# TheShadow29/vognet-pytorch

Hardware: AMD Instinct MI355X
Metric: queries/sec (VOGNet forward, gt5 spat, bs=4) (higher is better)
Workload: dtype bf16; 1 GPU; VOGNet spat gt5 (obj_tx+mul_tx, use_rel) bs=4; global_batch=4, batch_per_gpu=4, sentence_len=12, batches_in_flight=4, lang_cobatch=1, lstm=persistent layer kernel (1 launch per layer), submission=hipGraph on 4 HIP streams, weights=seeded default-init-like, vocab 5000, launches_per_forward=see kernels_usec (--full): steps joined by '+' share one launch (csrc/pair.hip)

## Files before the change

### include/vog_hip.h

```cpp
#ifndef VOG_HIP_H
#define VOG_HIP_H

#include <stddef.h>
#include <stdint.h>

#ifdef __cplusplus
extern "C" {
#endif

#define VOG_ABI_VERSION 1

typedef enum { VOG_BF16 = 0, VOG_F16 = 1 } vog_dtype;
typedef enum { VOG_MDL_IGRND = 0, VOG_MDL_VGRND = 1, VOG_MDL_VOG = 2 } vog_mdl_kind;
typedef enum { VOG_CONC_SEP = 0, VOG_CONC_TEMP = 1, VOG_CONC_SPAT = 2 } vog_conc_type;

int vog_version(void);
const char* vog_last_error(void);


struct vog_vislang_args;
typedef struct vog_gemm_args {
  const void* a; int a_is_f32; int64_t lda; const int32_t* a_rows;
  const void* w; int64_t ldw;
  const float* bias;
// ... 131 lines not shown
int vog_lang_prep(void* zero, int64_t zero_bytes, int64_t ones_bytes, const int64_t* words_ind, const int64_t* word_mask,
                  const int64_t* lens, int32_t* tok, int32_t* rows, int Bn, int T, int nsrl,
                  int seq_len, int vocab_size,
                  const void* emb16, void* a0_frag, int emb_dim, void* stream);

typedef struct vog_visprep_args {
  const float* src0; void* dst0; int64_t n0; const float* src1; void* dst1; int64_t n1; vog_dtype dtype;
  const float* props; int n_rows; float vid_w, vid_h;
  const float* w_pe0; float* u0; int H0; float nfrm_div0;
  const float* w_pe1; float* u1; int H1; float nfrm_div1;
} vog_visprep_args;
int vog_vis_prep(const vog_visprep_args* a, void* stream);
int vog_prep_fused(void* zero, int64_t zero_bytes, int64_t ones_bytes, const int64_t* words_ind, const int64_t* word_mask,
                   const int64_t* lens, int32_t* tok, int32_t* rows, int Bn, int T, int nsrl,
                   int seq_len, int vocab_size, const void* emb16, void* a0_frag, int emb_dim,
                   const vog_visprep_args* vis, void* stream);

typedef struct vog_lstm_step_args {
  const float* gx; const void* whh; const void* h_in; void* h_out; float* c;
  void* out16; const int64_t* lens; int Bn, T, R, step; vog_dtype dtype;
  int out_frag; int final_row0;
} vog_lstm_step_args;
int vog_bilstm_step(const vog_lstm_step_args* a, void* stream);
typedef struct vog_lstm_layer_args {
  const float* gxs; const void* whh; void* hx; uint32_t* sync; void* out16;
  const int64_t* lens; int Bn, T, R; vog_dtype dtype;
  int out_frag;
  const void* wih; const void* xa; const float* bias; int K;
  uint32_t* fault; int inject_stall;
  const float* gx_table; const int32_t* tok;
} vog_lstm_layer_args;
int vog_bilstm_layer_supported(int Bn, int R);
int vog_bilstm_fused_cols(void);
int64_t vog_bilstm_hx_bytes(int Bn, int T, int R);
int vog_bilstm_layer(const vog_lstm_layer_args* a, void* stream);

int vog_lstm_pack_whh(const float* whh_fwd, const float* whh_bwd, void* dst_host, int R, vog_dtype dtype);
int vog_lstm_pack_w(const float* w_fwd, const float* w_bwd, void* dst_host, int R, int K, vog_dtype dtype);

int vog_srl_argvec(const float* full, const int64_t* capture, const int64_t* inds_msk,
                   const float* w, const float* bias, float* lang,
                   int Bn, int T, int nsrl, int L, void* stream);

typedef struct vog_vislang_args {
  const float* vis; const float* lang; float* x32; void* x16;
  int n_vid, nfrm, nppf, nsrl, dv, dl; int lang_per_vid;
  int nc_v; vog_dtype dtype;
} vog_vislang_args;
int vog_vislang_layout(const vog_vislang_args* a, void* stream);

typedef struct vog_score_args {
  const float* h1; const float* w2; const float* b2;
  const int64_t* arg_msk; const int64_t* cmp_msk;
  float* outs; float* outs_eval;
  int n_vid, nfrm, nppf, nsrl, dh; int conc_type; int ncmp, nc_v, nvl, nfrm0, nppf0;
} vog_score_args;
int vog_score_head(const vog_score_args* a, void* stream);

typedef struct vog_predcmp_args {
  const float* final_hidden;
  const float* prop_seg;
  const float* w0; const float* b0; const float* w2; const float* b2;
  const float* outs;
  const int64_t* arg_msk; const int64_t* cmp_msk; const int64_t* verb_ind;
  float* vidf_outs; float* fin_scores_loss; float* fin_scores;
  int B, ncmp, nvl, nsrl, NP, nfrm0, nppf0, L, dp0, dps;
// ... 402 lines not shown
```

### vognet-pytorch_amd/csrc/lstm.hip

```cpp
#include <stdlib.h>
#include "lstm_dev.h"
#include "wpack_dev.h"
#include "pair_ids.h"

namespace vog {

__global__ void lstm_schedule_kernel(const int64_t* __restrict__ lens, int32_t* __restrict__ rows,
                                     int Bn, int T) {
  const int i = blockIdx.x * blockDim.x + threadIdx.x;
  if (i >= Bn * T) return;
  const int b = i / T, t = i % T;
  const int len = (int)lens[b];
  rows[i] = t < len ? t * Bn + b : -1;
  rows[Bn * T + i] = t < len ? T * Bn - 1 + (len - 1 - t) * Bn + b : -1;
}

const void* kid_lstm_layer_f16() { return reinterpret_cast<const void*>(lstm_layer_kernel<F16, 32>); }

int lstm_step_run(const vog_lstm_step_args* a, hipStream_t st) {
  VOG_CHECK_ARG(a && a->gx && a->whh && a->h_in && a->h_out && a->c && a->out16 && a->lens);
  VOG_CHECK_ARG(a->Bn > 0 && a->T > 0 && a->R > 0 && (a->R % 32) == 0 && a->step >= 0 && a->step < a->T);
  VOG_CHECK_ARG(a->h_in != a->h_out);
  LstmParams p{a->gx, (const unsigned short*)a->whh, (const unsigned short*)a->h_in,
               (unsigned short*)a->h_out, a->c, (unsigned short*)a->out16, a->lens,
               a->Bn, a->T, a->R, a->step, a->out_frag, a->final_row0, 0};
  static const int dbg = perf_env("VOG_LSTM_DEBUG") ? atoi(perf_env("VOG_LSTM_DEBUG")) : 0;
  p.debug = dbg;
  dim3 grid(ceil_div(a->R, 4), 2);
  VOG_DISPATCH_DTYPE(a->dtype, ::vog::launch((lstm_step_kernel<T16>), grid, dim3(256), 0, st, p));
  VOG_LAUNCH_CHECK();
  return 0;
}

}

extern "C" int vog_bilstm_step(const vog_lstm_step_args* a, void* stream) {
  return vog::lstm_step_run(a, (hipStream_t)stream);
}

extern "C" int vog_bilstm_layer_supported(int Bn, int R) {
  const int ks = R / 32;
  return Bn >= 1 && Bn <= 16 && R % 32 == 0 && R / 32 <= 64 && (ks == 1 || ks == 2 || ks == 4 || ks == 32);
}

extern "C" int vog_bilstm_fused_cols(void) { return 16 * vog::LstmLayerBody<vog::F16, 32>::NCT_MAX; }

extern "C" int64_t vog_bilstm_hx_bytes(int Bn, int T, int R) {
  if (Bn <= 0 || T <= 0 || R <= 0) return -1;
  return (int64_t)T * 2 * Bn * R * 2;
}

extern "C" int vog_bilstm_layer(const vog_lstm_layer_args* a, void* stream) {
  VOG_CHECK_ARG(a && (a->gxs || a->wih || a->gx_table) && a->whh && a->hx && a->sync && a->out16 && a->lens && a->T > 0);
  VOG_CHECK_ARG(!a->gx_table || (a->tok && a->Bn * a->T <= vog::LstmLayerBody<vog::F16, 32>::TOK_MAX));
  if (!vog_bilstm_layer_supported(a->Bn, a->R))
    VOG_FAIL(-1, "persistent BiLSTM layer: unsupported Bn=%d R=%d (use vog_bilstm_step)", a->Bn, a->R);
  vog::LstmLayerParams p{a->gxs, (const unsigned short*)a->whh, (unsigned short*)a->hx, a->sync,
                         (unsigned short*)a->out16, a->lens, a->Bn, a->T, a->R, a->out_frag,
                         (const unsigned short*)a->wih, (const unsigned short*)a->xa, a->bias, a->K,
                         a->fault, a->inject_stall, 0, a->gx_table, a->tok};
  if (const char* e = vog::perf_env("VOG_LSTM_HALF_PROJ")) p.half_proj = atoi(e);
  const bool fused = a->wih != nullptr && !a->gx_table;
  if (a->gx_table) p.wih = nullptr;
  if (fused) VOG_CHECK_ARG(a->xa && a->bias && a->K > 0 && (a->K % 256) == 0 && a->Bn * a->T <= vog_bilstm_fused_cols());
  dim3 grid(a->R / 32, 2);
  hipStream_t st = (hipStream_t)stream;
  size_t lds_extra = 0;
  if (const char* e = vog::perf_env("VOG_LSTM_LDS_EXTRA")) lds_extra = (size_t)atoi(e);
#define VOG_LAUNCH_LAYER(KS)                                                                          \
  VOG_DISPATCH_DTYPE(a->dtype, {                                                                      \
    auto kern = vog::lstm_layer_kernel<T16, KS>;                                                      \
    using Body = vog::LstmLayerBody<T16, KS>;                                                         \
    static bool attr_set = false;                                                                     \
    if (!attr_set) {                                                                                  \
      VOG_HIP(hipFuncSetAttribute(reinterpret_cast<const void*>(kern),                                \
                                  hipFuncAttributeMaxDynamicSharedMemorySize, 156 * 1024));          \
      attr_set = true;                                                                                \
    }                                                                                                 \
    ::vog::launch(kern, grid, dim3(512),                                                              \
                  (fused ? Body::lds_fused(a->Bn, a->Bn * a->T) : Body::lds_plain(a->Bn)) + lds_extra, st, p); \
  })
  switch (a->R / 32) {
    case 1: VOG_LAUNCH_LAYER(1); break;
    case 2: VOG_LAUNCH_LAYER(2); break;
    case 4: VOG_LAUNCH_LAYER(4); break;
    default: VOG_LAUNCH_LAYER(32); break;
  }
#undef VOG_LAUNCH_LAYER
  VOG_LAUNCH_CHECK();
  return 0;
}

extern "C" int vog_lstm_schedule(const int64_t* lens, int32_t* rows, int Bn, int T, void* stream) {
  VOG_CHECK_ARG(lens && rows && Bn > 0 && T > 0);
  ::vog::launch(vog::lstm_schedule_kernel, dim3(vog::ceil_div(Bn * T, 128)), dim3(128), 0,
                     (hipStream_t)stream, lens, rows, Bn, T);
  VOG_LAUNCH_CHECK();
  return 0;
}

extern "C" int vog_lstm_pack_whh(const float* whh_fwd, const float* whh_bwd, void* dst_host, int R,
                                 vog_dtype dtype) {
  return vog_lstm_pack_w(whh_fwd, whh_bwd, dst_host, R, R, dtype);
}

extern "C" int vog_lstm_pack_w(const float* whh_fwd, const float* whh_bwd, void* dst_host, int R, int K,
                               vog_dtype dtype) {
  VOG_CHECK_ARG(whh_fwd && whh_bwd && dst_host && R > 0 && (R % 4) == 0 && K > 0 && (K % 32) == 0);
  unsigned short* dst = (unsigned short*)dst_host;
  for (int64_t g = 0; g < (int64_t)8 * R * K / 8; ++g) {
    int n, k;
    vog::wpack_lstm_src(g, R, K, &n, &k);
    const float* src = (n < 4 * R ? whh_fwd : whh_bwd) + (int64_t)(n % (4 * R)) * K + k;
    unsigned short* d = dst + g * 8;
    for (int j = 0; j < 8; ++j) {
      if (dtype == VOG_BF16) {
        unsigned int u; memcpy(&u, &src[j], 4);
        u += 0x7fffu + ((u >> 16) & 1u);
        d[j] = (unsigned short)(u >> 16);
      } else {
        _Float16 h = (_Float16)src[j];
// ... 7 lines not shown
```

### vognet-pytorch_amd/csrc/lstm_dev.h

```cpp
#pragma once
#include "common.h"

namespace vog {

struct LstmParams {
  const float* gxs; const unsigned short* whh; const unsigned short* h_in; unsigned short* h_out;
  float* c; unsigned short* out16; const int64_t* lens;
  int Bn, T, R, step; int out_frag, final_row0; int debug;
};

__device__ __forceinline__ float sigm(float x) { return 1.0f / (1.0f + __expf(-x)); }
__device__ __forceinline__ float sigm_fast(float x) { return __builtin_amdgcn_rcpf(1.0f + __expf(-x)); }
__device__ __forceinline__ float tanh_fast(float x) {
  const float a = fabsf(x);
  const float e = __expf(-2.0f * a);
  const float t = (1.0f - e) * __builtin_amdgcn_rcpf(1.0f + e);
  return x < 0.f ? -t : t;
}
__device__ __forceinline__ float tanh_(float x) {
  const float a = fabsf(x);
  const float e = __expf(-2.0f * a);
  const float t = (1.0f - e) / (1.0f + e);
  return x < 0.f ? -t : t;
}
// ... 90 lines not shown
    VOG_TS(2);
  }
}

struct LstmLayerParams {
  const float* gxs; const unsigned short* whh; unsigned short* hx; unsigned int* sync;
  unsigned short* out16; const int64_t* lens; int Bn, T, R; int out_frag;
  const unsigned short* wih; const unsigned short* xa; const float* bias; int K;
  unsigned int* fault; int inject_stall;
  int half_proj;
  const float* gxtab; const int32_t* tok;
};

#define VOG_RLX_AGENT __ATOMIC_RELAXED, __HIP_MEMORY_SCOPE_AGENT
#define VOG_RLX_WG __ATOMIC_RELAXED, __HIP_MEMORY_SCOPE_WORKGROUP


__device__ __forceinline__ u32x4 load16_l2(const void* base, unsigned byte_off, unsigned bytes) {
  const __amdgpu_buffer_rsrc_t r = __builtin_amdgcn_make_buffer_rsrc(const_cast<void*>(base), 0, (int)bytes, 0x00020000);
  return __builtin_amdgcn_raw_buffer_load_b128(r, (int)byte_off, 0, 16 );
}
__device__ __forceinline__ bool has_unwritten(u32x4 v) {
  unsigned m = 0;
#pragma unroll
  for (int i = 0; i < 4; ++i) { const unsigned y = ~v[i]; m |= (y - 0x00010001u) & v[i] & 0x80008000u; }
  return m != 0;
}
__device__ __forceinline__ unsigned xcc_id() {
  unsigned x;
  asm volatile("s_getreg_b32 %0, hwreg(HW_REG_XCC_ID)" : "=s"(x));
  return x & 15u;
}

template <typename T16, int KSTEPS>
struct LstmLayerBody {
  using Params = LstmLayerParams;
  static constexpr int THREADS = 512;
  static constexpr int RW = KSTEPS * 32, HS_LD = RW + 32;
  static constexpr int GX_PITCH = 20;
  static constexpr int NCT_MAX = 5;
  static constexpr size_t gx_bytes(int ncols) { return (size_t)8 * ((ncols + 15) / 16 * 16) * GX_PITCH * 4; }
  static constexpr size_t GX_BYTES = gx_bytes(16 * NCT_MAX);
  static constexpr size_t hs_bytes(int Bn) { return ((size_t)2 * Bn * HS_LD * 2 + 15) / 16 * 16; }
  static constexpr size_t xbuf_bytes(int ncols) { return (size_t)2 * ((ncols + 15) / 16) * 8 * 1024; }
  static constexpr int TOK_MAX = 16 * 24;
  static constexpr size_t TAIL = 16 + 16 * 32 * 2 + TOK_MAX * 4;
  static constexpr size_t lds_plain(int Bn) { return hs_bytes(Bn) + TAIL; }
  static constexpr size_t lds_fused(int Bn, int ncols) {
    return gx_bytes(ncols) + (hs_bytes(Bn) > xbuf_bytes(ncols) ? hs_bytes(Bn) : xbuf_bytes(ncols)) + TAIL;
  }
  static constexpr size_t LDS_MAX = GX_BYTES + ((size_t)2 * 16 * HS_LD * 2 > (size_t)2 * NCT_MAX * 8 * 1024 ? (size_t)2 * 16 * HS_LD * 2 : (size_t)2 * NCT_MAX * 8 * 1024) + TAIL;

  static __device__ __forceinline__ void run(const LstmLayerParams& p, const BlockCtx& cx, unsigned char* smem) {
    const int tid = threadIdx.x, lane = tid & 63;
    const int wid = __builtin_amdgcn_readfirstlane(tid >> 6);
    const int dir = cx.by;
    const int R = p.R;
    const int tile0 = cx.bx * 8 + wid;
    const int b = lane & 15, ul = lane >> 4, kg = (lane >> 4) * 8;
    const bool valid_b = b < p.Bn;
    const int len = valid_b ? (int)p.lens[b] : 0;
    const bool fused = p.wih != nullptr;
    const int ncols = p.Bn * p.T;
    const int gx_cols = (ncols + 15) / 16 * 16;
    unsigned char* uni = smem + (fused ? gx_bytes(ncols) : 0);
    unsigned short* hs = reinterpret_cast<unsigned short*>(uni);
    const size_t uni_bytes = fused ? (hs_bytes(p.Bn) > xbuf_bytes(ncols) ? hs_bytes(p.Bn) : xbuf_bytes(ncols)) : hs_bytes(p.Bn);
    unsigned int* flags = reinterpret_cast<unsigned int*>(uni + uni_bytes);
    unsigned short* pub = reinterpret_cast<unsigned short*>(uni + uni_bytes + 16);
    int* tokl = reinterpret_cast<int*>(uni + uni_bytes + 16 + 16 * 32 * 2);
    const bool tab = p.gxtab != nullptr;
    const int unit0 = tile0 * 4 + ul;
    auto load_tab = [&](int s2, float (&g)[4], const int* tk) __attribute__((always_inline)) {
      int row = 0;
      const bool on = valid_b && s2 < len && s2 < p.T;
      if (on) row = tk[b * p.T + (dir == 0 ? s2 : len - 1 - s2)];
      const float4 v = *reinterpret_cast<const float4*>(p.gxtab + (((int64_t)row * 2 + dir) * R + unit0) * 4);
      g[0] = v.x; g[1] = v.y; g[2] = v.z; g[3] = v.w;
    };
    float gtA[4] = {0.f, 0.f, 0.f, 0.f}, gtB[4] = {0.f, 0.f, 0.f, 0.f}, gtC[4] = {0.f, 0.f, 0.f, 0.f};
    if (tab) {
      load_tab(0, gtA, p.tok);
      load_tab(1, gtB, p.tok);
      load_tab(2, gtC, p.tok);
      for (int i = tid; i < p.Bn * p.T; i += THREADS) tokl[i] = p.tok[i];
    }

    if (tid == 0) {
      flags[0] = 0;
      __hip_atomic_fetch_add(p.sync + 16 + dir * 16 + xcc_id(), 1u, VOG_RLX_AGENT);
    }

    float c = 0.f, h_own = 0.f;
    VOG_TSL(p.T, 0);
    float* gxl = reinterpret_cast<float*>(smem) + (size_t)wid * gx_cols * GX_PITCH;
    if (fused) {
      unsigned char* xch = uni;
      const int nct = (ncols + 15) >> 4;
      const int ksteps = p.K >> 5;
      const int nchunk = (p.half_proj && p.K >= 2048) ? (ksteps >> 4) : (ksteps >> 3);
      f32x4 ga[NCT_MAX];
#pragma unroll
      for (int ct = 0; ct < NCT_MAX; ++ct) ga[ct] = f32x4{0.f, 0.f, 0.f, 0.f};
      const u16x8* wsrc = reinterpret_cast<const u16x8*>(p.wih) + (((int64_t)dir * (R / 4) + tile0) * ksteps) * 64 + lane;
      const uint4* xsrc = reinterpret_cast<const uint4*>(p.xa);
      unsigned char* xbuf[2] = {xch, xch + nct * 8 * 1024};
      auto load_w = [&](u16x8 (&wq)[8], int c) {
#pragma unroll
        for (int ks = 0; ks < 8; ++ks) wq[ks] = wsrc[(c * 8 + ks) * 64];
      };
      auto dma_x = [&](int c) {
#pragma unroll
        for (int j = 0; j < NCT_MAX; ++j) {
          const int piece = j * 8 + wid;
          const int ct = piece >> 3, r = ((piece & 7) << 6) + lane;
          __builtin_amdgcn_global_load_lds(
              (const __attribute__((address_space(1))) void*)(xsrc + ((int64_t)(ct < nct ? ct : 0) * ksteps + c * 8) * 64 + r),
              (__attribute__((address_space(3))) void*)(xbuf[c & 1] + (ct < nct ? piece : (piece & 7)) * 1024), 16, 0, 0);
        }
      };
      auto mfmas = [&](const u16x8 (&wq)[8], int c) {
        const unsigned char* xb = xbuf[c & 1];
#pragma unroll
        for (int ct = 0; ct < NCT_MAX; ++ct)
          if (ct < nct) {
#pragma unroll
            for (int ks = 0; ks < 8; ++ks) {
              const u16x8 xf = *reinterpret_cast<const u16x8*>(xb + ((ct * 8 + ks) * 64 + lane) * 16);
              ga[ct] = mfma16<T16>(wq[ks], xf, ga[ct]);
            }
          }
      };
      u16x8 w0[8], w1[8];
      dma_x(0); load_w(w0, 0);
      if (nchunk > 1) { dma_x(1); load_w(w1, 1); }
      for (int c = 0; c < nchunk; c += 2) {
        if (c + 1 < nchunk) asm volatile("s_waitcnt vmcnt(%0)" ::"n"(NCT_MAX + 8) : "memory");
        else asm volatile("s_waitcnt vmcnt(0)" ::: "memory");
        __syncthreads();
        mfmas(w0, c);
        __syncthreads();
        if (c + 2 < nchunk) { dma_x(c + 2); load_w(w0, c + 2); }
        if (c + 1 < nchunk) {
          if (c + 2 < nchunk) asm volatile("s_waitcnt vmcnt(%0)" ::"n"(NCT_MAX + 8) : "memory");
          else asm volatile("s_waitcnt vmcnt(0)" ::: "memory");
          __syncthreads();
          mfmas(w1, c + 1);
          __syncthreads();
          if (c + 3 < nchunk) { dma_x(c + 3); load_w(w1, c + 3); }
        }
      }
      float bs[4];
#pragma unroll
      for (int r = 0; r < 4; ++r) bs[r] = p.bias[(int64_t)dir * 4 * R + (int64_t)r * R + tile0 * 4 + ul];
#pragma unroll
      for (int ct = 0; ct < NCT_MAX; ++ct)
        if (ct < nct)
          *reinterpret_cast<float4*>(gxl + (ct * 16 + b) * GX_PITCH + ul * 4) =
              make_float4(ga[ct][0] + bs[0], ga[ct][1] + bs[1], ga[ct][2] + bs[2], ga[ct][3] + bs[3]);
    }
    VOG_TSL(p.T, 1);
    u16x8 wf[KSTEPS];
#pragma unroll
    for (int ks = 0; ks < KSTEPS; ++ks)
      wf[ks] = *reinterpret_cast<const u16x8*>(
          p.whh + ((((int64_t)dir * (R / 4) + tile0) * KSTEPS + ks) * 64 + lane) * 8);
    bool dead = false;
    if (tid == 0) {
      unsigned spins = 0, nz = 0;
      for (;;) {
        unsigned sum = 0;
        nz = 0;
#pragma unroll
        for (int x = 0; x < 16; ++x) {
          const unsigned v = __hip_atomic_load(p.sync + 16 + dir * 16 + x, VOG_RLX_AGENT);
          sum += v;
          nz += v != 0 ? 1u : 0u;
        }
        if (sum >= cx.gx) break;
        __builtin_amdgcn_s_sleep(2);
        if (++spins > (1u << 20) || __hip_atomic_load(p.sync + 2, VOG_RLX_AGENT) != 0) {
          __hip_atomic_store(p.sync + 2, 1u, VOG_RLX_AGENT);
          flags[0] = 1;
          nz = 2;
          break;
        }
      }
      flags[1] = nz == 1 ? 1u : 0u;
    }
    __syncthreads();
    const bool same_xcd = flags[1] != 0;
    dead = flags[0] != 0 || p.inject_stall == 1 || (p.inject_stall == 2 && dir == 1);

    const unsigned hx_bytes = (unsigned)((size_t)p.T * 2 * p.Bn * R * 2);
    const int cps = RW / 8;
    const int nchunks = p.Bn * cps;
    const int hs_buf = p.Bn * HS_LD;

    for (int s = 0; s < p.T; ++s) {
      VOG_TSL(s, 0);
      float gin[4] = {0.f, 0.f, 0.f, 0.f};
      if (tab) {
#pragma unroll
        for (int r = 0; r < 4; ++r) { gin[r] = gtA[r]; gtA[r] = gtB[r]; gtB[r] = gtC[r]; }
        if (s == 0) load_tab(3, gtC, tokl);
      } else
      if (fused) {
        if (valid_b && s < len) {
          const int pos_in = dir == 0 ? s : len - 1 - s;
          const float4 g4 = *reinterpret_cast<const float4*>(gxl + (b * p.T + pos_in) * GX_PITCH + ul * 4);
          gin[0] = g4.x; gin[1] = g4.y; gin[2] = g4.z; gin[3] = g4.w;
        }
      } else {
#pragma unroll
        for (int r = 0; r < 4; ++r)
          gin[r] = valid_b ? p.gxs[(((int64_t)dir * p.T + s) * p.Bn + b) * 4 * R + (int64_t)r * R + tile0 * 4 + ul] : 0.f;
      }
      f32x4 acc0 = f32x4{0.f, 0.f, 0.f, 0.f}, acc1 = f32x4{0.f, 0.f, 0.f, 0.f};
      if (s > 0) {
        unsigned short* hsb = hs + (s & 1) * hs_buf;
        const unsigned slot_off = (unsigned)(((size_t)(s - 1) * 2 + dir) * p.Bn * R * 2);
        constexpr int MAXR = 4;
#ifndef VOG_LSTM_INFL
#define VOG_LSTM_INFL 4
#endif
        constexpr int INFL = VOG_LSTM_INFL;
        u32x4 vq[INFL];
        const int sb0 = tid / cps, j0 = tid - sb0 * cps;
        const unsigned off0 = slot_off + (unsigned)(sb0 * R + j0 * 8) * 2;
        const unsigned off_step = (unsigned)((THREADS / cps) * R) * 2;
        const int lds0 = sb0 * HS_LD + j0 * 8, lds_step = (THREADS / cps) * HS_LD;
        static_assert(THREADS % (RW / 8) == 0 || (RW / 8) % THREADS == 0, "hand-off fetch: chunk stride");
#pragma unroll
        for (int r0 = 0; r0 < MAXR; r0 += INFL) {
#pragma unroll
        for (int q = 0; q < INFL; ++q)
          if (tid + (r0 + q) * THREADS < nchunks) vq[q] = load16_l2(p.hx, off0 + (r0 + q) * off_step, hx_bytes);
#pragma unroll
        for (int q = 0; q < INFL; ++q) {
          const int r = r0 + q;
// ... 85 lines not shown
        } else {
          if (valid_b) pub[b * 32 + wid * 4 + ul] = x0;
          __syncthreads();
          if (tid < p.Bn * 4) {
            const int sb = tid >> 2, q = tid & 3;
            const u32x4 v = *reinterpret_cast<const u32x4*>(pub + sb * 32 + q * 8);
            u32x4* dst = reinterpret_cast<u32x4*>(slot + (size_t)sb * R + cx.bx * 32 + q * 8);
            asm volatile("global_store_dwordx4 %0, %1, off sc1" :: "v"(dst), "v"(v) : "memory");
          }
        }
      }
      VOG_TSL(s, 4);
    }
    if (dead && p.fault && tid == 0 &&
        __hip_atomic_exchange(p.sync + 3, 1u, __ATOMIC_RELAXED, __HIP_MEMORY_SCOPE_AGENT) == 0u)
      __hip_atomic_fetch_add(p.fault, 1u, __ATOMIC_RELAXED, __HIP_MEMORY_SCOPE_SYSTEM);
    if (valid_b) {
      const int unit = tile0 * 4 + ul;
      const unsigned short v = dead ? (unsigned short)0x7fff : to16<T16>(h_own);
      if (p.out_frag) p.out16[frag_a(p.Bn * p.T + b, dir * R + unit, 2 * R)] = v;
      else p.out16[((int64_t)p.Bn * p.T + b) * 2 * R + (int64_t)dir * R + unit] = v;
      if (dead)
        for (int t = 0; t < p.T; ++t) {
          if (p.out_frag) p.out16[frag_a(b * p.T + t, dir * R + unit, 2 * R)] = (unsigned short)0x7fff;
          else p.out16[((int64_t)b * p.T + t) * 2 * R + (int64_t)dir * R + unit] = (unsigned short)0x7fff;
        }
    }
  }
};

#ifndef VOG_LSTM_KATTR
#define VOG_LSTM_KATTR
#endif
template <typename T16, int KSTEPS>
__global__ __launch_bounds__(512) VOG_LSTM_KATTR void lstm_layer_kernel(LstmLayerParams p) {
  extern __shared__ __attribute__((aligned(16))) unsigned char lstm_smem[];
  LstmLayerBody<T16, KSTEPS>::run(p, BlockCtx{blockIdx.x, blockIdx.y, gridDim.x, gridDim.y}, lstm_smem);
}

}
```

### vognet-pytorch_amd/csrc/pair.hip

```cpp
#include <functional>
#include <map>
#include <mutex>
#include <utility>
#include "gemm_dev.h"
#include "lstm_dev.h"
#include "txtail_dev.h"
#include "visenc_dev.h"
#include "qkvrb_dev.h"
#include <tuple>
#include "pair_ids.h"

#ifndef VOG_VS_PAIR_DEPTH
#define VOG_VS_PAIR_DEPTH 2
#endif

namespace vog {

thread_local std::vector<LaunchRecord>* g_pair_capture = nullptr;

template <typename A, typename B>
__global__ __launch_bounds__((A::THREADS > B::THREADS ? A::THREADS : B::THREADS))
void pair_kernel(typename A::Params a, typename B::Params b, unsigned nA, unsigned gax, unsigned gay,
                 unsigned gbx, unsigned gby, unsigned delay_b) {
  extern __shared__ __attribute__((aligned(1024))) unsigned char pair_smem[];
// ... 17 lines not shown
      ra.arg_bytes != sizeof(typename A::Params) || rb.arg_bytes != sizeof(typename B::Params))
    VOG_FAIL(-1, "pair launch: recorded launches do not match the registered bodies");
  typename A::Params pa; typename B::Params pb;
  memcpy(&pa, ra.args, sizeof(pa));
  memcpy(&pb, rb.args, sizeof(pb));
  const unsigned nA = ra.grid[0] * ra.grid[1], nB = rb.grid[0] * rb.grid[1];
  const size_t lds = ra.dyn_lds > rb.dyn_lds ? ra.dyn_lds : rb.dyn_lds;
  if (lds > 156 * 1024) VOG_FAIL(-1, "pair launch: %zu bytes of LDS", lds);
  auto kern = pair_kernel<A, B>;
  static bool attr_set = false;
  if (!attr_set) {
    VOG_HIP(hipFuncSetAttribute(reinterpret_cast<const void*>(kern), hipFuncAttributeMaxDynamicSharedMemorySize,
                                156 * 1024));
    attr_set = true;
  }
  static const unsigned delay_b = perf_env("VOG_PAIR_DELAY") ? (unsigned)atoi(perf_env("VOG_PAIR_DELAY")) : 0u;
  ::vog::launch(kern, dim3(nA + nB), dim3(MAXT), lds, st, pa, pb, nA, ra.grid[0], ra.grid[1], rb.grid[0], rb.grid[1], delay_b);
  VOG_LAUNCH_CHECK();
  return 0;
}

using SkinnyIh = GemmSkinnyBody<F16, false, 4, 1, 4>;
using SkinnyRow = GemmSkinnyRowBody<F16, 8>;
template <typename B>
static int launch_pair_outproj(const LaunchRecord& ra, const LaunchRecord& rb, hipStream_t st) {
  GemmParams pa;
  if (ra.arg_bytes == sizeof(pa)) {
    memcpy(&pa, ra.args, sizeof(pa));
    if (SkinnyRow::fits(pa, ra.grid[1])) return launch_pair<SkinnyRow, B>(ra, rb, st);
  }
  return launch_pair<SkinnyIh, B>(ra, rb, st);
}

static constexpr int kPairDeclined = 1;
static std::map<std::pair<const void*, const void*>, PairFn>& registry() {
  static std::map<std::pair<const void*, const void*>, PairFn> r;
  static std::once_flag once;
  std::call_once(once, [] {
    using Lstm = LstmLayerBody<F16, 32>;
    r[{kid_lstm_layer_f16(), kid_vis_enc_f16()}] = &launch_pair<Lstm, VisEncBody<F16>>;
    r[{kid_lstm_layer_f16(), kid_vis_enc_stream_f16()}] = &launch_pair<Lstm, VisEncStreamBody<F16, VOG_VS_PAIR_DEPTH>>;
    r[{kid_lstm_layer_f16(), kid_gemm_pipe_qkv(VOG_BF16)}] = &launch_pair<Lstm, GemmPipeBody<BF16, 64, 64, 2, EPI_QKV>>;
    r[{kid_lstm_layer_f16(), kid_gemm_pipe_qkv(VOG_F16)}] = &launch_pair<Lstm, GemmPipeBody<F16, 64, 64, 2, EPI_QKV>>;
    r[{kid_lstm_layer_f16(), kid_tx_tail_512(VOG_BF16)}] = &launch_pair<Lstm, TxTailBody<BF16, F16, 2, false, 0>>;
    r[{kid_lstm_layer_f16(), kid_tx_tail_512(VOG_F16)}] = &launch_pair<Lstm, TxTailBody<F16, F16, 2, false, 0>>;
    r[{kid_lstm_layer_f16(), kid_vis_enc_stream_split_f16()}] = &launch_pair<Lstm, VisEncStreamBody<F16, VOG_VS_DEPTH, true>>;
    r[{kid_lstm_layer_f16(), kid_tx_tail_split_512_f16()}] = &launch_pair<Lstm, TxTailBody<F16, F16, 2, false, 0, 1, true>>;
    r[{kid_gemm_skinny_f16(), kid_gemm_pipe_qkv_split_f16()}] = &launch_pair_outproj<GemmPipeBody<F16, 64, 64, 2, EPI_QKV, true>>;
    r[{kid_gemm_skinny_f16(), kid_gemm_pipe_qkv(VOG_BF16)}] = &launch_pair_outproj<GemmPipeBody<BF16, 64, 64, 2, EPI_QKV>>;
    r[{kid_gemm_skinny_f16(), kid_gemm_pipe_qkv(VOG_F16)}] = &launch_pair_outproj<GemmPipeBody<F16, 64, 64, 2, EPI_QKV>>;
    r[{kid_gemm_pipe_plain3_f16(), kid_gemm_pipe_qkv(VOG_BF16)}] = &launch_pair<GemmPipeBody<F16, 64, 64, 3, EPI_PLAIN>, GemmPipeBody<BF16, 64, 64, 2, EPI_QKV>>;
    r[{kid_gemm_pipe_plain3_f16(), kid_gemm_pipe_qkv(VOG_F16)}] = &launch_pair<GemmPipeBody<F16, 64, 64, 3, EPI_PLAIN>, GemmPipeBody<F16, 64, 64, 2, EPI_QKV>>;
  });
  return r;
}

int pair_launch(const std::function<int(hipStream_t)>& fa, const std::function<int(hipStream_t)>& fb,
                hipStream_t st, bool* fused) {
  if (fused) *fused = false;
  std::vector<LaunchRecord> recs;
  if (g_pair_capture) { VOG_TRY(fa(st)); return fb(st); }
  g_pair_capture = &recs;
  int rc = fa(st);
  const size_t na = recs.size();
  if (rc == 0) rc = fb(st);
  g_pair_capture = nullptr;
  if (rc != 0) return rc;
  if (na == 1 && recs.size() == 2) {
    auto it = registry().find({recs[0].host_fn, recs[1].host_fn});
    if (it != registry().end()) {
      const int prc = it->second(recs[0], recs[1], st);
      if (prc != kPairDeclined) {
        if (fused) *fused = prc == 0;
        return prc;
      }
    }
  }
  VOG_TRY(fa(st));
  return fb(st);
}
// ... 3 lines not shown
```

### vognet-pytorch_amd/csrc/pair_ids.h

```cpp
#pragma once
namespace vog {
const void* kid_gemm_skinny_f16();
const void* kid_gemm_skinny_wide_f16();
const void* kid_gemm_skinny_f32a_short(int dtype);
const void* kid_gemm_pipe_qkv(int dtype);
const void* kid_gemm_pipe_plain3_f16();
const void* kid_lstm_layer_f16();
const void* kid_tx_tail_512(int dtype);
const void* kid_vis_enc_f16();
const void* kid_vis_enc_stream_f16();
const void* kid_gemm_pipe_qkv_split_f16();
const void* kid_tx_tail_split_512_f16();
const void* kid_vis_enc_stream_split_f16();
}
```

### vognet-pytorch_amd/lib.py

```python
from __future__ import annotations

import ctypes as C
import os
from typing import Optional

_HERE = os.path.dirname(os.path.abspath(__file__))
LIB_PATH = os.environ.get("VOG_HIP_LIB") or os.path.join(_HERE, "csrc", "libvog_hip.so")

VOG_BF16, VOG_F16 = 0, 1
MDL_KIND = {"igrnd": 0, "vgrnd": 1, "vog": 2}
CONC_TYPE = {"sep": 0, "svsq": 0, "temp": 1, "spat": 2}
DTYPE = {"bf16": VOG_BF16, "f16": VOG_F16, "fp16": VOG_F16}

c_i32, c_i64, c_f32, c_vp = C.c_int, C.c_int64, C.c_float, C.c_void_p


class VogError(RuntimeError):
    pass


class GemmArgs(C.Structure):
    _fields_ = [("a", c_vp), ("a_is_f32", c_i32), ("lda", c_i64), ("a_rows", c_vp),
                ("w", c_vp), ("ldw", c_i64), ("bias", c_vp), ("residual", c_vp), ("ldr", c_i64),
                ("c32", c_vp), ("c16", c_vp), ("ldc", c_i64), ("ldc16", c_i64),
# ... 324 lines not shown

AVG_EMA, AVG_SWA = 1, 2


class OptAvgTensor(C.Structure):
    _fields_ = [("avg", c_vp), ("p", c_vp), ("n", c_i64)]


class OptAvgState(C.Structure):
    _fields_ = [("n_averaged", c_i32), ("updated", c_i32), ("w", c_f32), ("reserved", c_i32)]


class OptAvgArgs(C.Structure):
    _fields_ = [("tensors", C.POINTER(OptAvgTensor)), ("n_tensors", c_i32), ("mode", c_i32), ("decay", C.c_double),
                ("warmup", c_i32), ("start", c_i32), ("every", c_i32), ("opt_state", c_vp), ("step", c_i32), ("state", c_vp)]


class Batch(C.Structure):
    _fields_ = [("B", c_i32), ("ncmp", c_i32), ("T", c_i32),
                ("srl_arg_words_ind", c_vp), ("srl_arg_word_mask", c_vp),
                ("srl_arg_word_mask_len", c_vp), ("srl_arg_words_capture", c_vp),
                ("srl_arg_inds_msk", c_vp), ("num_cmp_msk", c_vp), ("verb_ind_in_srl", c_vp),
                ("pad_region_feature", c_vp), ("seg_feature_for_frms", c_vp), ("pad_proposals", c_vp),
                ("mdl_outs", c_vp), ("mdl_outs_eval", c_vp), ("vidf_outs", c_vp),
                ("fin_scores_loss", c_vp), ("fin_scores", c_vp), ("pred_rec", c_vp),
                ("shared_lang", c_vp), ("shared_final_hidden", c_vp), ("fault", c_vp), ("obj_out", c_vp), ("stats", c_vp),
                ("enc_prop", c_vp), ("enc_seg", c_vp)]


SYMBOLS = {
    "vog_version": (c_i32, []),
    "vog_ctx_split_supported": (c_i32, [c_vp, c_i32]),
    "vog_bilstm_fused_cols": (c_i32, []),
    "vog_last_error": (C.c_char_p, []),
    "vog_gemm_bias_act": (c_i32, [C.POINTER(GemmArgs), c_vp]),
    "vog_pack_w_frag": (c_i32, [c_vp, c_i64, c_i32, c_i32, c_vp, c_i32]),
    "vog_pack_w_frag32": (c_i32, [c_vp, c_i64, c_i32, c_i32, c_vp, c_i32]),
    "vog_tx_tail_supported": (c_i32, [c_i32, c_i32, c_i32]),
    "vog_tx_tail_scratch_bytes": (c_i64, [c_i32, c_i32]),
    "vog_tx_tail_fwd": (c_i32, [C.POINTER(TxTailArgs), c_vp]),
    "vog_encoder_layer_fwd": (c_i32, [C.POINTER(EncoderLayerArgs), c_vp]),
    "vog_vis_encode_supported": (c_i32, [c_i32, c_i32, c_i32, c_i32]),
    "vog_vis_encode": (c_i32, [C.POINTER(VisencArgs), c_vp]),
    "vog_seg_replicate": (c_i32, [C.POINTER(VisencArgs), c_vp]),
    "vog_vis_concat": (c_i32, [C.POINTER(VisconcatArgs), c_vp]),
    "vog_obj_restore": (c_i32, [C.POINTER(ObjrestoreArgs), c_vp]),
    "vog_loss_scratch_bytes": (c_i64, [C.POINTER(LossArgs)]),
    "vog_loss_fwd": (c_i32, [C.POINTER(LossArgs), c_vp]),
    "vog_loss_bwd": (c_i32, [C.POINTER(LossArgs), c_vp, c_vp, c_vp]),
    "vog_assemble_batch": (c_i32, [C.POINTER(AssembleArgs), c_vp]),
    "vog_assemble_from_bank": (c_i32, [C.POINTER(BankAssembleArgs), c_vp]),
    "vog_splitk_finish": (c_i32, [C.POINTER(SplitkProb), C.POINTER(SplitkProb), c_vp]),
    "vog_qkv_proj": (c_i32, [C.POINTER(QkvArgs), c_vp]),
    "vog_qkv_rowblock_supported": (c_i32, [c_i32, c_i32]),
    "vog_qkv_combine": (c_i32, [C.POINTER(QkvCombArgs), c_vp]),
    "vog_rel_attention_fwd": (c_i32, [C.POINTER(AttnArgs), c_vp]),
    "vog_rel_attention_struct_fwd": (c_i32, [C.POINTER(AttnStructArgs), c_vp]),
    "vog_residual_layernorm": (c_i32, [c_vp, c_vp, c_vp, c_vp, c_vp, c_i32, c_i32, c_i32, c_vp]),
    "vog_cast_f32_to_t16": (c_i32, [c_vp, c_vp, c_i64, c_vp, c_vp, c_i64, c_i32, c_vp]),
    "vog_box_u": (c_i32, [c_vp, c_vp, c_vp, c_i32, c_i32, c_f32, c_f32, c_f32, c_vp]),
    "vog_srl_gather": (c_i32, [c_vp, c_vp, c_vp, c_i32, c_i32, c_i32, c_i32, c_i32, c_vp]),
    "vog_bilstm_layer_supported": (c_i32, [c_i32, c_i32]),
    "vog_mul_tail_bwd_scratch_bytes": (c_i64, [c_i32, c_i32, c_i32, c_i32]),
    "vog_mul_tail_bwd": (c_i32, [C.POINTER(TailBwdArgs), c_vp]),
    "vog_attn_f32_scratch_bytes": (c_i64, [c_i32, c_i32, c_i32, c_i32]),
    "vog_attn_f32": (c_i32, [C.POINTER(AttnF32Args), c_vp]),
# ... 131 lines not shown
```

Baseline: 65630 queries/s.

## Specialize fused BiLSTM projection on column-tile count and stage x through registers

Makes the number of projection column tiles a template parameter of the persistent BiLSTM layer kernel, with one instantiation per tile count, so the register accumulators and MFMA loops are sized exactly and runtime guards disappear. The input-projection x operand is now loaded into registers and written to LDS instead of using global_load_lds DMA with explicit vmcnt waits. The K loop is restructured to drop one barrier per chunk and adds sched_barrier hints plus optional nontemporal weight loads. The pairing registry is extended to cover every instantiation. This costs more compiled kernel variants, and register staging of x raises register pressure.

```diff
diff --git a/include/vog_hip.h b/include/vog_hip.h
--- a/include/vog_hip.h
+++ b/include/vog_hip.h
@@ -187,6 +187,7 @@
 } vog_lstm_layer_args;
 int vog_bilstm_layer_supported(int Bn, int R);
 int vog_bilstm_fused_cols(void);
+int vog_bilstm_fused_tiles(int cols);
 int64_t vog_bilstm_hx_bytes(int Bn, int T, int R);
 int vog_bilstm_layer(const vog_lstm_layer_args* a, void* stream);
 
diff --git a/vognet-pytorch_amd/csrc/lstm.hip b/vognet-pytorch_amd/csrc/lstm.hip
--- a/vognet-pytorch_amd/csrc/lstm.hip
+++ b/vognet-pytorch_amd/csrc/lstm.hip
@@ -15,7 +15,22 @@
   rows[Bn * T + i] = t < len ? T * Bn - 1 + (len - 1 - t) * Bn + b : -1;
 }
 
-const void* kid_lstm_layer_f16() { return reinterpret_cast<const void*>(lstm_layer_kernel<F16, 32>); }
+int lstm_layer_nct(int cols) {
+  constexpr int NCT_MAX = LstmLayerBody<F16, 32>::NCT_MAX;
+  return cols >= 1 && cols <= 16 * NCT_MAX ? (cols + 15) / 16 : 0;
+}
+
+const void* kid_lstm_layer_f16(int nct) {
+  switch (nct) {
+    case 0: return reinterpret_cast<const void*>(lstm_layer_kernel<F16, 32, 0>);
+    case 1: return reinterpret_cast<const void*>(lstm_layer_kernel<F16, 32, 1>);
+    case 2: return reinterpret_cast<const void*>(lstm_layer_kernel<F16, 32, 2>);
+    case 3: return reinterpret_cast<const void*>(lstm_layer_kernel<F16, 32, 3>);
+    case 4: return reinterpret_cast<const void*>(lstm_layer_kernel<F16, 32, 4>);
+    case 5: return reinterpret_cast<const void*>(lstm_layer_kernel<F16, 32, 5>);
+    default: return nullptr;
+  }
+}
 
 int lstm_step_run(const vog_lstm_step_args* a, hipStream_t st) {
   VOG_CHECK_ARG(a && a->gx && a->whh && a->h_in && a->h_out && a->c && a->out16 && a->lens);
@@ -45,6 +60,11 @@
 
 extern "C" int vog_bilstm_fused_cols(void) { return 16 * vog::LstmLayerBody<vog::F16, 32>::NCT_MAX; }
 
+extern "C" int vog_bilstm_fused_tiles(int cols) {
+  const int nct = vog::lstm_layer_nct(cols);
+  return nct > 0 ? nct : -1;
+}
+
 extern "C" int64_t vog_bilstm_hx_bytes(int Bn, int T, int R) {
   if (Bn <= 0 || T <= 0 || R <= 0) return -1;
   return (int64_t)T * 2 * Bn * R * 2;
@@ -63,14 +83,16 @@
   const bool fused = a->wih != nullptr && !a->gx_table;
   if (a->gx_table) p.wih = nullptr;
   if (fused) VOG_CHECK_ARG(a->xa && a->bias && a->K > 0 && (a->K % 256) == 0 && a->Bn * a->T <= vog_bilstm_fused_cols());
+  const int nct = fused ? vog::lstm_layer_nct(a->Bn * a->T) : 0;
+  if (fused && nct == 0) VOG_FAIL(-1, "persistent BiLSTM layer: no fused instantiation for %d columns", a->Bn * a->T);
   dim3 grid(a->R / 32, 2);
   hipStream_t st = (hipStream_t)stream;
   size_t lds_extra = 0;
   if (const char* e = vog::perf_env("VOG_LSTM_LDS_EXTRA")) lds_extra = (size_t)atoi(e);
-#define VOG_LAUNCH_LAYER(KS)                                                                          \
+#define VOG_LAUNCH_LAYER_NCT(KS, NCT)                                                                 \
   VOG_DISPATCH_DTYPE(a->dtype, {                                                                      \
-    auto kern = vog::lstm_layer_kernel<T16, KS>;                                                      \
-    using Body = vog::LstmLayerBody<T16, KS>;                                                         \
+    auto kern = vog::lstm_layer_kernel<T16, KS, NCT>;                                                 \
+    using Body = vog::LstmLayerBody<T16, KS, NCT>;                                                    \
     static bool attr_set = false;                                                                     \
     if (!attr_set) {                                                                                  \
       VOG_HIP(hipFuncSetAttribute(reinterpret_cast<const void*>(kern),                                \
@@ -80,6 +102,15 @@
     ::vog::launch(kern, grid, dim3(512),                                                              \
                   (fused ? Body::lds_fused(a->Bn, a->Bn * a->T) : Body::lds_plain(a->Bn)) + lds_extra, st, p); \
   })
+#define VOG_LAUNCH_LAYER(KS)                     \
+  switch (nct) {                                 \
+    case 0: VOG_LAUNCH_LAYER_NCT(KS, 0); break;  \
+    case 1: VOG_LAUNCH_LAYER_NCT(KS, 1); break;  \
+    case 2: VOG_LAUNCH_LAYER_NCT(KS, 2); break;  \
+    case 3: VOG_LAUNCH_LAYER_NCT(KS, 3); break;  \
+    case 4: VOG_LAUNCH_LAYER_NCT(KS, 4); break;  \
+    default: VOG_LAUNCH_LAYER_NCT(KS, 5); break; \
+  }
   switch (a->R / 32) {
     case 1: VOG_LAUNCH_LAYER(1); break;
     case 2: VOG_LAUNCH_LAYER(2); break;
@@ -87,6 +118,7 @@
     default: VOG_LAUNCH_LAYER(32); break;
   }
 #undef VOG_LAUNCH_LAYER
+#undef VOG_LAUNCH_LAYER_NCT
   VOG_LAUNCH_CHECK();
   return 0;
 }
diff --git a/vognet-pytorch_amd/csrc/lstm_dev.h b/vognet-pytorch_amd/csrc/lstm_dev.h
--- a/vognet-pytorch_amd/csrc/lstm_dev.h
+++ b/vognet-pytorch_amd/csrc/lstm_dev.h
@@ -146,13 +146,26 @@
   return x & 15u;
 }
 
-template <typename T16, int KSTEPS>
+#ifndef VOG_LSTM_NT_WIH
+#define VOG_LSTM_NT_WIH 0
+#endif
+#ifndef VOG_LSTM_NT_WHH
+#define VOG_LSTM_NT_WHH 0
+#endif
+template <bool NT>
+__device__ __forceinline__ u16x8 load_wfrag(const u16x8* src) {
+  if constexpr (NT) return __builtin_nontemporal_load(src);
+  else return *src;
+}
+
+template <typename T16, int KSTEPS, int NCT = 0>
 struct LstmLayerBody {
   using Params = LstmLayerParams;
   static constexpr int THREADS = 512;
   static constexpr int RW = KSTEPS * 32, HS_LD = RW + 32;
   static constexpr int GX_PITCH = 20;
   static constexpr int NCT_MAX = 5;
+  static_assert(NCT >= 0 && NCT <= NCT_MAX, "column tiles of the fused projection");
   static constexpr size_t gx_bytes(int ncols) { return (size_t)8 * ((ncols + 15) / 16 * 16) * GX_PITCH * 4; }
   static constexpr size_t GX_BYTES = gx_bytes(16 * NCT_MAX);
   static constexpr size_t hs_bytes(int Bn) { return ((size_t)2 * Bn * HS_LD * 2 + 15) / 16 * 16; }
@@ -174,16 +187,16 @@
     const int b = lane & 15, ul = lane >> 4, kg = (lane >> 4) * 8;
     const bool valid_b = b < p.Bn;
     const int len = valid_b ? (int)p.lens[b] : 0;
-    const bool fused = p.wih != nullptr;
+    constexpr bool fused = NCT > 0;
     const int ncols = p.Bn * p.T;
-    const int gx_cols = (ncols + 15) / 16 * 16;
+    constexpr int gx_cols = NCT * 16;
     unsigned char* uni = smem + (fused ? gx_bytes(ncols) : 0);
     unsigned short* hs = reinterpret_cast<unsigned short*>(uni);
     const size_t uni_bytes = fused ? (hs_bytes(p.Bn) > xbuf_bytes(ncols) ? hs_bytes(p.Bn) : xbuf_bytes(ncols)) : hs_bytes(p.Bn);
     unsigned int* flags = reinterpret_cast<unsigned int*>(uni + uni_bytes);
     unsigned short* pub = reinterpret_cast<unsigned short*>(uni + uni_bytes + 16);
     int* tokl = reinterpret_cast<int*>(uni + uni_bytes + 16 + 16 * 32 * 2);
-    const bool tab = p.gxtab != nullptr;
+    const bool tab = !fused && p.gxtab != nullptr;
     const int unit0 = tile0 * 4 + ul;
     auto load_tab = [&](int s2, float (&g)[4], const int* tk) __attribute__((always_inline)) {
       int row = 0;
@@ -208,77 +221,84 @@
     float c = 0.f, h_own = 0.f;
     VOG_TSL(p.T, 0);
     float* gxl = reinterpret_cast<float*>(smem) + (size_t)wid * gx_cols * GX_PITCH;
-    if (fused) {
+    if constexpr (fused) {
       unsigned char* xch = uni;
-      const int nct = (ncols + 15) >> 4;
+      constexpr int nct = NCT;
       const int ksteps = p.K >> 5;
       const int nchunk = (p.half_proj && p.K >= 2048) ? (ksteps >> 4) : (ksteps >> 3);
-      f32x4 ga[NCT_MAX];
-#pragma unroll
-      for (int ct = 0; ct < NCT_MAX; ++ct) ga[ct] = f32x4{0.f, 0.f, 0.f, 0.f};
+      f32x4 ga[nct];
+#pragma unroll
+      for (int ct = 0; ct < nct; ++ct) ga[ct] = f32x4{0.f, 0.f, 0.f, 0.f};
       const u16x8* wsrc = reinterpret_cast<const u16x8*>(p.wih) + (((int64_t)dir * (R / 4) + tile0) * ksteps) * 64 + lane;
-      const uint4* xsrc = reinterpret_cast<const uint4*>(p.xa);
+      float bs[4];
+#pragma unroll
+      for (int r = 0; r < 4; ++r) bs[r] = p.bias[(int64_t)dir * 4 * R + (int64_t)r * R + tile0 * 4 + ul];
       unsigned char* xbuf[2] = {xch, xch + nct * 8 * 1024};
       auto load_w = [&](u16x8 (&wq)[8], int c) {
 #pragma unroll
-        for (int ks = 0; ks < 8; ++ks) wq[ks] = wsrc[(c * 8 + ks) * 64];
-      };
-      auto dma_x = [&](int c) {
-#pragma unroll
-        for (int j = 0; j < NCT_MAX; ++j) {
-          const int piece = j * 8 + wid;
-          const int ct = piece >> 3, r = ((piece & 7) << 6) + lane;
-          __builtin_amdgcn_global_load_lds(
-              (const __attribute__((address_space(1))) void*)(xsrc + ((int64_t)(ct < nct ? ct : 0) * ksteps + c * 8) * 64 + r),
-              (__attribute__((address_space(3))) void*)(xbuf[c & 1] + (ct < nct ? piece : (piece & 7)) * 1024), 16, 0, 0);
-        }
+        for (int ks = 0; ks < 8; ++ks) wq[ks] = load_wfrag<VOG_LSTM_NT_WIH != 0>(wsrc + (c * 8 + ks) * 64);
       };
       auto mfmas = [&](const u16x8 (&wq)[8], int c) {
         const unsigned char* xb = xbuf[c & 1];
 #pragma unroll
-        for (int ct = 0; ct < NCT_MAX; ++ct)
-          if (ct < nct) {
-#pragma unroll
-            for (int ks = 0; ks < 8; ++ks) {
-              const u16x8 xf = *reinterpret_cast<const u16x8*>(xb + ((ct * 8 + ks) * 64 + lane) * 16);
-              ga[ct] = mfma16<T16>(wq[ks], xf, ga[ct]);
-            }
-          }
+        for (int ct = 0; ct < nct; ++ct) {
+#pragma unroll
+          for (int ks = 0; ks < 8; ++ks) {
+            const u16x8 xf = *reinterpret_cast<const u16x8*>(xb + ((ct * 8 + ks) * 64 + lane) * 16);
+            ga[ct] = mfma16<T16>(wq[ks], xf, ga[ct]);
+          }
+          __builtin_amdgcn_sched_barrier(0);
+        }
       };
       u16x8 w0[8], w1[8];
-      dma_x(0); load_w(w0, 0);
-      if (nchunk > 1) { dma_x(1); load_w(w1, 1); }
-      for (int c = 0; c < nchunk; c += 2) {
-        if (c + 1 < nchunk) asm volatile("s_waitcnt vmcnt(%0)" ::"n"(NCT_MAX + 8) : "memory");
-        else asm volatile("s_waitcnt vmcnt(0)" ::: "memory");
-        __syncthreads();
-        mfmas(w0, c);
-        __syncthreads();
-        if (c + 2 < nchunk) { dma_x(c + 2); load_w(w0, c + 2); }
-        if (c + 1 < nchunk) {
-          if (c + 2 < nchunk) asm volatile("s_waitcnt vmcnt(%0)" ::"n"(NCT_MAX + 8) : "memory");
-          else asm volatile("s_waitcnt vmcnt(0)" ::: "memory");
-          __syncthreads();
-          mfmas(w1, c + 1);
-          __syncthreads();
-          if (c + 3 < nchunk) { dma_x(c + 3); load_w(w1, c + 3); }
-        }
-      }
-      float bs[4];
-#pragma unroll
-      for (int r = 0; r < 4; ++r) bs[r] = p.bias[(int64_t)dir * 4 * R + (int64_t)r * R + tile0 * 4 + ul];
-#pragma unroll
-      for (int ct = 0; ct < NCT_MAX; ++ct)
-        if (ct < nct)
-          *reinterpret_cast<float4*>(gxl + (ct * 16 + b) * GX_PITCH + ul * 4) =
-              make_float4(ga[ct][0] + bs[0], ga[ct][1] + bs[1], ga[ct][2] + bs[2], ga[ct][3] + bs[3]);
+      u32x4 x0[nct], x1[nct];
+      const u32x4* xreg = reinterpret_cast<const u32x4*>(p.xa) + (wid << 6) + lane;
+      auto load_x = [&](u32x4 (&xq)[nct], int c) {
+#pragma unroll
+        for (int ct = 0; ct < nct; ++ct) xq[ct] = xreg[((int64_t)ct * ksteps + c * 8) * 64];
+      };
+      auto put_x = [&](const u32x4 (&xq)[nct], int c) {
+#pragma unroll
+        for (int ct = 0; ct < nct; ++ct) *reinterpret_cast<u32x4*>(xbuf[c & 1] + (ct * 8 + wid) * 1024 + lane * 16) = xq[ct];
+      };
+      auto chunk0 = [&](int c) { put_x(x0, c); __syncthreads(); mfmas(w0, c); };
+      auto chunk1 = [&](int c) { put_x(x1, c); __syncthreads(); mfmas(w1, c); };
+#define VOG_KEEP_BIAS() asm volatile("" ::"v"(bs[0]), "v"(bs[1]), "v"(bs[2]), "v"(bs[3]))
+      load_x(x0, 0); load_w(w0, 0);
+      if (nchunk == 1) {
+        VOG_KEEP_BIAS();
+        chunk0(0);
+      } else {
+        load_x(x1, 1); load_w(w1, 1);
+        VOG_KEEP_BIAS();
+        int c = 0;
+        for (; c + 3 < nchunk; c += 2) {
+          chunk0(c);
+          load_x(x0, c + 2); load_w(w0, c + 2);
+          chunk1(c + 1);
+          load_x(x1, c + 3); load_w(w1, c + 3);
+        }
+        chunk0(c);
+        if (c + 2 < nchunk) {
+          load_x(x0, c + 2); load_w(w0, c + 2);
+          chunk1(c + 1);
+          chunk0(c + 2);
+        } else {
+          chunk1(c + 1);
+        }
+      }
+#undef VOG_KEEP_BIAS
+#pragma unroll
+      for (int ct = 0; ct < nct; ++ct)
+        *reinterpret_cast<float4*>(gxl + (ct * 16 + b) * GX_PITCH + ul * 4) =
+            make_float4(ga[ct][0] + bs[0], ga[ct][1] + bs[1], ga[ct][2] + bs[2], ga[ct][3] + bs[3]);
     }
     VOG_TSL(p.T, 1);
     u16x8 wf[KSTEPS];
 #pragma unroll
     for (int ks = 0; ks < KSTEPS; ++ks)
-      wf[ks] = *reinterpret_cast<const u16x8*>(
-          p.whh + ((((int64_t)dir * (R / 4) + tile0) * KSTEPS + ks) * 64 + lane) * 8);
+      wf[ks] = load_wfrag<VOG_LSTM_NT_WHH != 0>(reinterpret_cast<const u16x8*>(
+          p.whh + ((((int64_t)dir * (R / 4) + tile0) * KSTEPS + ks) * 64 + lane) * 8));
     bool dead = false;
     if (tid == 0) {
       unsigned spins = 0, nz = 0;
@@ -319,7 +339,7 @@
         for (int r = 0; r < 4; ++r) { gin[r] = gtA[r]; gtA[r] = gtB[r]; gtB[r] = gtC[r]; }
         if (s == 0) load_tab(3, gtC, tokl);
       } else
-      if (fused) {
+      if constexpr (fused) {
         if (valid_b && s < len) {
           const int pos_in = dir == 0 ? s : len - 1 - s;
           const float4 g4 = *reinterpret_cast<const float4*>(gxl + (b * p.T + pos_in) * GX_PITCH + ul * 4);
@@ -471,10 +491,10 @@
 #ifndef VOG_LSTM_KATTR
 #define VOG_LSTM_KATTR
 #endif
-template <typename T16, int KSTEPS>
+template <typename T16, int KSTEPS, int NCT = 0>
 __global__ __launch_bounds__(512) VOG_LSTM_KATTR void lstm_layer_kernel(LstmLayerParams p) {
   extern __shared__ __attribute__((aligned(16))) unsigned char lstm_smem[];
-  LstmLayerBody<T16, KSTEPS>::run(p, BlockCtx{blockIdx.x, blockIdx.y, gridDim.x, gridDim.y}, lstm_smem);
-}
-
-}
+  LstmLayerBody<T16, KSTEPS, NCT>::run(p, BlockCtx{blockIdx.x, blockIdx.y, gridDim.x, gridDim.y}, lstm_smem);
+}
+
+}
diff --git a/vognet-pytorch_amd/csrc/pair.hip b/vognet-pytorch_amd/csrc/pair.hip
--- a/vognet-pytorch_amd/csrc/pair.hip
+++ b/vognet-pytorch_amd/csrc/pair.hip
@@ -73,20 +73,39 @@
   return launch_pair<SkinnyIh, B>(ra, rb, st);
 }
 
+template <typename B>
+static int launch_pair_lstm(const LaunchRecord& ra, const LaunchRecord& rb, hipStream_t st) {
+  LstmLayerParams pa;
+  if (ra.arg_bytes != sizeof(pa)) VOG_FAIL(-1, "pair launch: recorded launch is not a BiLSTM layer");
+  memcpy(&pa, ra.args, sizeof(pa));
+  const int nct = pa.wih ? lstm_layer_nct(pa.Bn * pa.T) : 0;
+  if (ra.host_fn != kid_lstm_layer_f16(nct)) VOG_FAIL(-1, "pair launch: BiLSTM layer recorded with another tile count than %d", nct);
+  switch (nct) {
+    case 0: return launch_pair<LstmLayerBody<F16, 32, 0>, B>(ra, rb, st);
+    case 1: return launch_pair<LstmLayerBody<F16, 32, 1>, B>(ra, rb, st);
+    case 2: return launch_pair<LstmLayerBody<F16, 32, 2>, B>(ra, rb, st);
+    case 3: return launch_pair<LstmLayerBody<F16, 32, 3>, B>(ra, rb, st);
+    case 4: return launch_pair<LstmLayerBody<F16, 32, 4>, B>(ra, rb, st);
+    default: return launch_pair<LstmLayerBody<F16, 32, 5>, B>(ra, rb, st);
+  }
+}
+
 static constexpr int kPairDeclined = 1;
 static std::map<std::pair<const void*, const void*>, PairFn>& registry() {
   static std::map<std::pair<const void*, const void*>, PairFn> r;
   static std::once_flag once;
   std::call_once(once, [] {
-    using Lstm = LstmLayerBody<F16, 32>;
-    r[{kid_lstm_layer_f16(), kid_vis_enc_f16()}] = &launch_pair<Lstm, VisEncBody<F16>>;
-    r[{kid_lstm_layer_f16(), kid_vis_enc_stream_f16()}] = &launch_pair<Lstm, VisEncStreamBody<F16, VOG_VS_PAIR_DEPTH>>;
-    r[{kid_lstm_layer_f16(), kid_gemm_pipe_qkv(VOG_BF16)}] = &launch_pair<Lstm, GemmPipeBody<BF16, 64, 64, 2, EPI_QKV>>;
-    r[{kid_lstm_layer_f16(), kid_gemm_pipe_qkv(VOG_F16)}] = &launch_pair<Lstm, GemmPipeBody<F16, 64, 64, 2, EPI_QKV>>;
-    r[{kid_lstm_layer_f16(), kid_tx_tail_512(VOG_BF16)}] = &launch_pair<Lstm, TxTailBody<BF16, F16, 2, false, 0>>;
-    r[{kid_lstm_layer_f16(), kid_tx_tail_512(VOG_F16)}] = &launch_pair<Lstm, TxTailBody<F16, F16, 2, false, 0>>;
-    r[{kid_lstm_layer_f16(), kid_vis_enc_stream_split_f16()}] = &launch_pair<Lstm, VisEncStreamBody<F16, VOG_VS_DEPTH, true>>;
-    r[{kid_lstm_layer_f16(), kid_tx_tail_split_512_f16()}] = &launch_pair<Lstm, TxTailBody<F16, F16, 2, false, 0, 1, true>>;
+    for (int nct = 0; nct <= LstmLayerBody<F16, 32>::NCT_MAX; ++nct) {
+      const void* lstm = kid_lstm_layer_f16(nct);
+      r[{lstm, kid_vis_enc_f16()}] = &launch_pair_lstm<VisEncBody<F16>>;
+      r[{lstm, kid_vis_enc_stream_f16()}] = &launch_pair_lstm<VisEncStreamBody<F16, VOG_VS_PAIR_DEPTH>>;
+      r[{lstm, kid_gemm_pipe_qkv(VOG_BF16)}] = &launch_pair_lstm<GemmPipeBody<BF16, 64, 64, 2, EPI_QKV>>;
+      r[{lstm, kid_gemm_pipe_qkv(VOG_F16)}] = &launch_pair_lstm<GemmPipeBody<F16, 64, 64, 2, EPI_QKV>>;
+      r[{lstm, kid_tx_tail_512(VOG_BF16)}] = &launch_pair_lstm<TxTailBody<BF16, F16, 2, false, 0>>;
+      r[{lstm, kid_tx_tail_512(VOG_F16)}] = &launch_pair_lstm<TxTailBody<F16, F16, 2, false, 0>>;
+      r[{lstm, kid_vis_enc_stream_split_f16()}] = &launch_pair_lstm<VisEncStreamBody<F16, VOG_VS_DEPTH, true>>;
+      r[{lstm, kid_tx_tail_split_512_f16()}] = &launch_pair_lstm<TxTailBody<F16, F16, 2, false, 0, 1, true>>;
+    }
     r[{kid_gemm_skinny_f16(), kid_gemm_pipe_qkv_split_f16()}] = &launch_pair_outproj<GemmPipeBody<F16, 64, 64, 2, EPI_QKV, true>>;
     r[{kid_gemm_skinny_f16(), kid_gemm_pipe_qkv(VOG_BF16)}] = &launch_pair_outproj<GemmPipeBody<BF16, 64, 64, 2, EPI_QKV>>;
     r[{kid_gemm_skinny_f16(), kid_gemm_pipe_qkv(VOG_F16)}] = &launch_pair_outproj<GemmPipeBody<F16, 64, 64, 2, EPI_QKV>>;
diff --git a/vognet-pytorch_amd/csrc/pair_ids.h b/vognet-pytorch_amd/csrc/pair_ids.h
--- a/vognet-pytorch_amd/csrc/pair_ids.h
+++ b/vognet-pytorch_amd/csrc/pair_ids.h
@@ -5,7 +5,8 @@
 const void* kid_gemm_skinny_f32a_short(int dtype);
 const void* kid_gemm_pipe_qkv(int dtype);
 const void* kid_gemm_pipe_plain3_f16();
-const void* kid_lstm_layer_f16();
+const void* kid_lstm_layer_f16(int nct);
+int lstm_layer_nct(int cols);
 const void* kid_tx_tail_512(int dtype);
 const void* kid_vis_enc_f16();
 const void* kid_vis_enc_stream_f16();
diff --git a/vognet-pytorch_amd/lib.py b/vognet-pytorch_amd/lib.py
--- a/vognet-pytorch_amd/lib.py
+++ b/vognet-pytorch_amd/lib.py
@@ -380,6 +380,7 @@
     "vog_version": (c_i32, []),
     "vog_ctx_split_supported": (c_i32, [c_vp, c_i32]),
     "vog_bilstm_fused_cols": (c_i32, []),
+    "vog_bilstm_fused_tiles": (c_i32, [c_i32]),
     "vog_last_error": (C.c_char_p, []),
     "vog_gemm_bias_act": (c_i32, [C.POINTER(GemmArgs), c_vp]),
     "vog_pack_w_frag": (c_i32, [c_vp, c_i64, c_i32, c_i32, c_vp, c_i32]),
```

Result: no change. 65560 queries/s (-0.1%).
